# allenai/satlas-super-resolution

Hardware: AMD Instinct MI355X
Metric: G+D train-step images/sec (higher is better)
Workload: dtype fp32h

## Files before the change

### satlas_super_resolution_amd/csrc/conv_x3r.hip

```cpp
#include "conv_x3r_core.h"
#include "conv_dispatch.h"

#ifdef SSR_PROBE
#define RPROBE(cond, k) do { if (cond) g_probe[(blockIdx.y * gridDim.x + blockIdx.x) * 16 + (k)] = __builtin_amdgcn_s_memtime(); } while (0)
#else
#define RPROBE(cond, k)
#endif

namespace {

template <int NTW, int NU, int EP, int TH = 8, int AM = 0>
__global__ __launch_bounds__((XrT<NTW, NU, TH>::NTHR)) void conv_x3r_kernel(const ssr_conv_desc d) {
    constexpr bool EX = AM == 1, H = AM == 2;
    using T = XrT<NTW, NU, TH>;
    constexpr int NT = NTW, NTT = T::NTT, NMF = T::NMF, BN = T::BN, WR = T::WR, MT = T::MT;
    constexpr int G_NPIX = T::NPIX, G_SUB = T::SUB, G_PV = T::PV, G_NPV = T::NPV;
    extern __shared__ __attribute__((aligned(16))) char smem[];
    int* ctl = reinterpret_cast<int*>(smem + T::CTL);
    const int ctl_addr = (int)(size_t)(__attribute__((address_space(3))) char*)(smem + T::CTL);
    const int tid = threadIdx.x, lane = tid & 63, wave = __builtin_amdgcn_readfirstlane(tid >> 6);
    const int tiles_x = (d.Gw + 15) / 16, tiles_y = (d.Gh + TH - 1) / TH;
    int b = blockIdx.x;
    const int tx_i = b % tiles_x; b /= tiles_x;
    const int ty_i = b % tiles_y;
    const int n = b / tiles_y;
    const int gy0 = ty_i * TH, gx0 = tx_i * 16;
    const int co0 = blockIdx.y * BN;
    const int Cin = d.Cin, Cin2 = d.Cin2;
    const int nchunks = (Cin + Cin2 + 15) / 16;
    const int cout_pad = d.CoutPad;
    const int tapstride = cout_pad * 64, wchunk = 9 * tapstride;
    RPROBE(tid == 0, 0);
    if (tid < 4 + NMF) ctl[tid] = 0;
    __syncthreads();

    f32x16 acc[MT][NT];
#pragma unroll
    for (int t = 0; t < MT; ++t)
#pragma unroll
        for (int u = 0; u < NT; ++u)
#pragma unroll
            for (int r = 0; r < 16; ++r) acc[t][u][r] = 0.f;

    if (wave >= NMF) {
        const int pw = wave - NMF;
        const int pt = tid - 64 * NMF;
#ifdef XR_PRIO
        __builtin_amdgcn_s_setprio(3);
#endif
        const int part = pt & 3, p4 = pt >> 2;
        int ppix[G_NPV];
#pragma unroll
        for (int q = 0; q < G_NPV; ++q) {
            const int pix = p4 + 64 * q;
            const int py = pix / XR_PW, px = pix - py * XR_PW;
            const int ly = gy0 + py - d.pad_y, lx = gx0 + px - d.pad_x;
            const bool okp = pix < G_NPIX && ly >= 0 && ly < d.Hi && lx >= 0 && lx < d.Wi;
            ppix[q] = okp ? (n * d.Hi + ly) * d.Wi + lx : -1;
        }
        const int plo0 = p4 * XR_ROWB + part * 8;
        const long xbytes = (long)d.N * d.Hi * d.Wi * 4;
        const void* xp = d.x.p;
        const void* x2p = d.x2.p ? d.x2.p : d.x.p;
        const int x_cs = d.x.cs, x_coff = d.x.coff, x2_cs = d.x2.p ? d.x2.cs : d.x.cs, x2_coff = d.x2.p ? d.x2.coff : d.x.coff;
        u32x4 rq[XR_PQ][G_NPV];
        auto load_chunk = [&](int c, auto jc) {
            constexpr int j = decltype(jc)::value;
            const bool live = c < nchunks;
            const int c0 = c * 16;
            const bool in_x = c0 < Cin;
            const int cb = in_x ? c0 : c0 - Cin, clim = live ? (in_x ? Cin : Cin2) : 0;
            const int cs = in_x ? x_cs : x2_cs, coff = in_x ? x_coff : x2_coff;
            const __amdgpu_buffer_rsrc_t rs = xr_rsrc(in_x ? xp : x2p, xbytes * cs);
            const int k = cb + part * 4;
#pragma unroll
            for (int q = 0; q < G_NPV; ++q) {
                const int off = (ppix[q] * cs + coff + k) * 4;
                const bool okl = (k < clim) & (ppix[q] >= 0);
#ifdef XR_X_NOXLOAD
                rq[j][q] = u32x4{(unsigned)off, (unsigned)okl, 0u, 0u};
#else
                rq[j][q] = __builtin_amdgcn_raw_buffer_load_b128(rs, okl ? off : XR_OOB, 0, 0);
#endif
            }
        };
        static_for<0, XR_PQ>([&](auto jc) { __builtin_amdgcn_sched_barrier(0); load_chunk(decltype(jc)::value, jc); __builtin_amdgcn_sched_barrier(0); });
        RPROBE(pt == 0, 8);
        int cfree = XR_NS;
        for (int c0 = 0; c0 < nchunks; c0 += XR_PQ) {
            static_for<0, XR_PQ>([&](auto jc) {
                constexpr int j = decltype(jc)::value;
                const int c = c0 + j;
                if (c < nchunks) {
                    if (c >= cfree) {
                        int spin = 0;
                        for (; spin < XR_SPIN_MAX; ++spin) {
                            cfree = xr_minN<NMF>(ctl_addr + 16) + XR_NS;
                            if (c < cfree) break;
                            __builtin_amdgcn_s_sleep(2);
                        }
                        if (spin == XR_SPIN_MAX) __builtin_trap();
                    }
                    char* base = smem + (c % XR_NS) * G_SUB;
#pragma unroll
                    for (int q = 0; q < G_NPV; ++q) {
#ifdef XR_X_NOSTORE
                        asm volatile("" :: "v"(rq[j][q]));
                        continue;
#endif
                        if constexpr (EX) {
                            if (q < G_NPV - 1 || pt < G_PV - (G_NPV - 1) * 256)
                                *reinterpret_cast<u32x4*>(base + p4 * XR_ROWB + part * 16 + q * 64 * XR_ROWB) = rq[j][q];
                        } else {
                            uint2 hi, lo;
                            split_f32x4<H>(rq[j][q], hi, lo);
                            if (q < G_NPV - 1 || pt < G_PV - (G_NPV - 1) * 256) {
                                *reinterpret_cast<uint2*>(base + plo0 + q * 64 * XR_ROWB) = hi;
                                *reinterpret_cast<uint2*>(base + plo0 + q * 64 * XR_ROWB + 32) = lo;
                            }
                        }
                    }
                    asm volatile("" ::: "memory");
                    if (lane == 0) *(xr_lds_int)(uintptr_t)(ctl_addr + 4 * pw) = c + 1;
                    asm volatile("" ::: "memory");
#if defined(XR_PRIO) && XR_PRIO == 1
                    if (c == 0) __builtin_amdgcn_s_setprio(0);
#endif
                }
                __builtin_amdgcn_sched_barrier(0);
                load_chunk(c + XR_PQ, jc);
                __builtin_amdgcn_sched_barrier(0);
            });
        }
        RPROBE(pt == 0, 9);
    } else {
        const int w = wave & 3, ug = wave >> 2;
        const int i = lane & 31, gq = lane >> 5;
        const int a_lane = ((i >> 4) * XR_PW + epi_col<XR_ROT>(i)) * XR_ROWB + gq * 16;
        const __amdgpu_buffer_rsrc_t rsw = xr_rsrc(d.w, (long)nchunks * wchunk);
        const int w_lane = (co0 + 32 * NTW * ug + i) * 64 + gq * 16;
        const int nitems = 3 * nchunks;
        const int nj = nitems > w ? (nitems - w + 3) / 4 : 0;
        const int glast = w + 4 * (nj - 1);
        if (nj == 0) {
            if (lane == 0) *(xr_lds_int)(uintptr_t)(ctl_addr + 16 + 4 * wave) = 0x3fffffff;
        } else {
            bf16x8 wf[WR][NT][2];
            constexpr int TPS = T::TPS, SPT = T::SPT, NSUB = 3 * SPT, NSETS = T::NSETS, PD = NSETS - 1;
            bf16x8 af[NSETS][TPS][2];
            auto load_w = [&](int g_, auto kxc, auto sc) {
                constexpr int kx = decltype(kxc)::value, s = decltype(sc)::value;
                const int gg = g_ < glast ? g_ : glast;
                const int c = gg / 3, ky = gg - 3 * c;
                const int off = c * wchunk + (ky * 3 + kx) * tapstride + w_lane;
#pragma unroll
                for (int u = 0; u < NT; ++u) {
                    wf[s][u][0] = __builtin_bit_cast(bf16x8, __builtin_amdgcn_raw_buffer_load_b128(rsw, off + u * 2048, 0, 0));
                    wf[s][u][1] = __builtin_bit_cast(bf16x8, __builtin_amdgcn_raw_buffer_load_b128(rsw, off + u * 2048 + 32, 0, 0));
                }
            };
            auto issue_a = [&](int base, auto qc, auto sc, auto hc) {
                constexpr int q = decltype(qc)::value, kx = q / SPT, part = q % SPT, s = decltype(sc)::value, H = decltype(hc)::value;
#pragma unroll
                for (int t2 = 0; t2 < TPS; ++t2)
                    af[s][t2][H] = *reinterpret_cast<const bf16x8*>(smem + base + kx * XR_ROWB + (part * TPS + t2) * XR_TILEB + 32 * H);
            };
            int avail = 0;
            auto ensure = [&](int c) {
                if (avail > c) return;
                int spin = 0;
                for (; spin < XR_SPIN_MAX; ++spin) {
                    avail = xr_min4(ctl_addr);
                    if (avail > c) break;
                    __builtin_amdgcn_s_sleep(1);
                }
                if (spin == XR_SPIN_MAX) __builtin_trap();
            };
            auto base_of = [&](int g_) { const int c = g_ / 3, ky = g_ - 3 * c; return (c % XR_NS) * G_SUB + ky * XR_PW * XR_ROWB + a_lane; };
            using I0 = std::integral_constant<int, 0>;
            using I1 = std::integral_constant<int, 1>;
#ifndef XR_WPRE
#define XR_WPRE 99
#endif
            constexpr int WPRE = XR_WPRE < WR ? XR_WPRE : WR;
            static_for<0, WPRE>([&](auto sc) {
                constexpr int s = decltype(sc)::value;
                __builtin_amdgcn_sched_barrier(0);
                load_w(w + 4 * (s / 3), std::integral_constant<int, s % 3>{}, sc);
                __builtin_amdgcn_sched_barrier(0);
            });
            RPROBE(tid == 0, 1);
            int g = w, c_cur = g / 3;
            int base_cur = base_of(g);
            ensure(c_cur);
            static_for<WPRE, WR>([&](auto sc) {
                constexpr int s = decltype(sc)::value;
                __builtin_amdgcn_sched_barrier(0);
                load_w(w + 4 * (s / 3), std::integral_constant<int, s % 3>{}, sc);
                __builtin_amdgcn_sched_barrier(0);
            });
            RPROBE(tid == 0, 2);
            static_for<0, PD>([&](auto qc) {
                issue_a(base_cur, qc, std::integral_constant<int, decltype(qc)::value % NSETS>{}, I1{});
                issue_a(base_cur, qc, std::integral_constant<int, decltype(qc)::value % NSETS>{}, I0{});
            });
            int gn = g + 4 < glast ? g + 4 : glast;
            int c_next = gn / 3, base_next = base_of(gn);
            int gnn = gn, c_nn = c_next, base_nn = base_next;
            auto body = [&](int j, auto jpc) {
                constexpr int JP = decltype(jpc)::value;
                static_for<0, NSUB>([&](auto qc) {
                    constexpr int q = decltype(qc)::value, kx = q / SPT, part = q % SPT, qn = q + PD;
                    constexpr int ws = (JP * 3 + kx) % WR, as = (JP * NSUB + q) % NSETS, asn = (JP * NSUB + qn) % NSETS;
                    auto group = [&](auto pc) {
                        constexpr int P = decltype(pc)::value;
                        if constexpr (EX) {
                            constexpr int H = P == 0 ? 1 : 0, S0 = P == 2 ? 2 : 0, S1 = P == 1 ? 2 : 4;
#pragma unroll
                            for (int sidx = S0; sidx < S1; ++sidx)
#pragma unroll
                                for (int t2 = 0; t2 < TPS; ++t2)
#pragma unroll
                                    for (int u = 0; u < NT; ++u) {
                                        const f32x4 av = __builtin_bit_cast(f32x4, af[as][t2][H]), bv = __builtin_bit_cast(f32x4, wf[ws][u][H]);
                                        acc[part * TPS + t2][u] = __builtin_amdgcn_mfma_f32_32x32x2f32(av[sidx], bv[sidx], acc[part * TPS + t2][u], 0, 0, 0);
                                    }
                        } else {
#pragma unroll
                            for (int t2 = 0; t2 < TPS; ++t2)
#pragma unroll
                                for (int u = 0; u < NT; ++u)
                                    acc[part * TPS + t2][u] = split_mfma<H>(af[as][t2][P == 0 ? 1 : 0], wf[ws][u][P == 1 ? 1 : 0], acc[part * TPS + t2][u]);
                        }
                    };
                    auto reads = [&](auto hc) {
#ifndef XR_X_NOA
                        if constexpr (qn < NSUB) issue_a(base_cur, std::integral_constant<int, qn>{}, std::integral_constant<int, asn>{}, hc);
                        else issue_a(base_next, std::integral_constant<int, qn - NSUB>{}, std::integral_constant<int, asn>{}, hc);
#endif
                    };
                    __builtin_amdgcn_sched_barrier(0);
                    if constexpr (qn == NSUB) {
                        if (c_next > c_cur) {
                            asm volatile("" ::: "memory");
                            if (lane == 0) *(xr_lds_int)(uintptr_t)(ctl_addr + 16 + 4 * wave) = c_next;
                            asm volatile("" ::: "memory");
                        }
                        ensure(c_next);
                        __builtin_amdgcn_sched_barrier(0);
                    }
                    group(std::integral_constant<int, 0>{});
                    __builtin_amdgcn_sched_barrier(0);
                    reads(I1{});
                    if constexpr (part == 0) {
#ifndef XR_X_NOW
                        constexpr int wsp = (JP * 3 + kx + WR - 1) % WR, ioff = (kx + WR - 1) / 3, tap = (kx + WR - 1) % 3;
                        load_w(g + 4 * ioff, std::integral_constant<int, tap>{}, std::integral_constant<int, wsp>{});
#endif
                    }
                    __builtin_amdgcn_sched_barrier(0);
                    group(std::integral_constant<int, 1>{});
                    __builtin_amdgcn_sched_barrier(0);
                    reads(I0{});
                    if constexpr (q == 0) {
                        gnn = g + 8 < glast ? g + 8 : glast;
                        c_nn = gnn / 3;
                        base_nn = base_of(gnn);
                    }
                    __builtin_amdgcn_sched_barrier(0);
                    group(std::integral_constant<int, 2>{});
                    __builtin_amdgcn_sched_barrier(0);
                });
                g += 4;
                c_cur = c_next; base_cur = base_next;
                gn = gnn; c_next = c_nn; base_next = base_nn;
#ifdef SSR_PROBE
                if (j < 5) RPROBE(tid == 0, 3 + j);
#endif
            };
            if constexpr (WR == 6 || (NSUB % NSETS) != 0) {
                for (int j = 0; j < nj; j += 2) {
                    body(j, std::integral_constant<int, 0>{});
                    if (j + 1 < nj) body(j + 1, std::integral_constant<int, 1>{});
                }
            } else {
                for (int j = 0; j < nj; ++j) body(j, std::integral_constant<int, 0>{});
            }
            asm volatile("" ::: "memory");
            if (lane == 0) *(xr_lds_int)(uintptr_t)(ctl_addr + 16 + 4 * wave) = 0x3fffffff;
        }
    }
    __syncthreads();
    RPROBE(tid == 0, 10);

    const bool is_mfma = wave < NMF;
    const int me = is_mfma ? (wave & 3) : wave - NMF;
    const int ut = is_mfma ? NTW * (wave >> 2) : 1;
#ifndef XR_X_NORED
    if (is_mfma) {
#pragma unroll
        for (int t = 0; t < MT; ++t)
#pragma unroll
            for (int u = 0; u < NT; ++u)
                if (!(t == me && u == 0)) {
                    char* sp = smem + ((me * MT + t) * NTT + ut + u) * XR_SLOT + lane * 16;
#pragma unroll
                    for (int q = 0; q < 4; ++q) {
                        f32x4 v = {acc[t][u][4 * q], acc[t][u][4 * q + 1], acc[t][u][4 * q + 2], acc[t][u][4 * q + 3]};
                        *reinterpret_cast<f32x4*>(sp + q * 1024) = v;
                    }
                }
    }
#endif
    __syncthreads();
    if ((is_mfma || NTW == 2) && me < MT) {
        f32x16 own;
#pragma unroll
        for (int r = 0; r < 16; ++r) own[r] = 0.f;
        if (is_mfma) {
#pragma unroll
            for (int t = 0; t < MT; ++t)
                if (t == me) own = acc[t][0];
        }
        f32x16 sum;
#pragma unroll
        for (int s = 0; s < 4; ++s) {
            f32x16 part;
            const char* sp = smem + ((s * MT + me) * NTT + ut) * XR_SLOT + lane * 16;
#ifdef XR_X_NORED
            part = own;
            asm volatile("" : "+v"(part));
#else
#pragma unroll
            for (int q = 0; q < 4; ++q) {
                const f32x4 v = *reinterpret_cast<const f32x4*>(sp + q * 1024);
                part[4 * q] = v[0]; part[4 * q + 1] = v[1]; part[4 * q + 2] = v[2]; part[4 * q + 3] = v[3];
            }
#endif
            const bool mine = is_mfma && s == me;
#pragma unroll
            for (int r = 0; r < 16; ++r) {
                const float p = mine ? own[r] : part[r];
                sum[r] = s == 0 ? p : sum[r] + p;
            }
        }
        if constexpr (H) {
#pragma unroll
            for (int r = 0; r < 16; ++r) sum[r] *= SSR_F32H_UNSCALE;
        }
        char* slab = smem + (((is_mfma ? me : 0) * MT + me) * NTT + ut) * XR_SLOT;
        const int cb = co0 + 32 * ut;
#ifdef XR_X_NOEPI
        float keep = 0.f;
#pragma unroll
        for (int r = 0; r < 16; ++r) keep += sum[r];
        if (keep == 123.456f) reinterpret_cast<float*>(d.y.p)[tid] = keep;
#else
        if constexpr (EP == XR_EP_GENERIC) conv_epilogue<float, XR_ROT>(d, sum, cb, n, gy0 + 2 * me, gx0, lane, slab);
        else xr_epilogue<EP>(d, sum, cb, n, gy0 + 2 * me, gx0, lane, slab);
#endif
    }
    RPROBE(tid == 0, 11);
}

template <int NTW, int NU, int EP, int TH = 8, int AM = 0>
int launch_x3r(const ssr_conv_desc& d, hipStream_t st) {
    using T = XrT<NTW, NU, TH>;
    auto kern = conv_x3r_kernel<NTW, NU, EP, TH, AM>;
    static bool attr_done[SSR_MAX_DEVICES] = {};
    const int dev = ssr_device_ordinal();
    if (!attr_done[dev]) {
        hipError_t e = hipFuncSetAttribute(reinterpret_cast<const void*>(kern), hipFuncAttributeMaxDynamicSharedMemorySize, T::LDS);
        if (e != hipSuccess) return (int)e;
        attr_done[dev] = true;
    }
    const int tiles = ((d.Gw + 15) / 16) * ((d.Gh + TH - 1) / TH) * d.N;
    hipLaunchKernelGGL(kern, dim3(tiles, d.CoutPad / T::BN, 1), dim3(T::NTHR), T::LDS, st, d);
    SSR_LAUNCH_CHECK();
    return SSR_OK;
}

int xr_pick_epilogue(const ssr_conv_desc& d) {
    static const bool generic_only = ssr_env_off("SSR_X3R_EPI");
    if (generic_only) return XR_EP_GENERIC;
    const long lim = 0x7fffff00L, npx = (long)d.N * d.Ho * d.Wo * 4;
    auto vok = [&](const ssr_view& v) { return (v.cs % 4) == 0 && (v.coff % 4) == 0 && ((uintptr_t)v.p % 16) == 0 && npx * v.cs <= lim; };
    if (d.fix_list || d.y0.p || d.y1.p || d.accumulate || d.m_relu || (d.Cout % 4) != 0 || !vok(d.y)) return XR_EP_GENERIC;
    if (d.oys != 1 || d.oxs != 1 || d.oyo != 0 || d.oxo != 0 || d.Ho < d.Gh || d.Wo < d.Gw) return XR_EP_GENERIC;
    const bool r1 = d.r1.p != nullptr, r2 = d.r2.p != nullptr, m = d.m.p != nullptr;
    if (d.act == SSR_ACT_LRELU && d.alpha == 1.f && !r1 && !r2 && !m) return XR_EP_LRELU;
    if (d.act == SSR_ACT_NONE && !m && (!r1 || (d.r1_nc >= d.Cout && vok(d.r1))) && (!r2 || (d.r2_nc >= d.Cout && vok(d.r2)))) return XR_EP_LIN;
    if (d.act == SSR_ACT_NONE && d.alpha == 1.f && m && !r1 && !r2 && d.m_c0 == 0 && d.m_c1 >= d.Cout && vok(d.m)) return XR_EP_MASK;
    return XR_EP_GENERIC;
}

template <int NTW, int NU, int TH = 8, int AM = 0>
int launch_x3r_ep(const ssr_conv_desc& d, hipStream_t st) {
    switch (xr_pick_epilogue(d)) {
        case XR_EP_LRELU: return launch_x3r<NTW, NU, XR_EP_LRELU, TH, AM>(d, st);
        case XR_EP_LIN: return launch_x3r<NTW, NU, XR_EP_LIN, TH, AM>(d, st);
        case XR_EP_MASK: return launch_x3r<NTW, NU, XR_EP_MASK, TH, AM>(d, st);
        default: return launch_x3r<NTW, NU, XR_EP_GENERIC, TH, AM>(d, st);
    }
}

int xr_tile_height(const ssr_conv_desc& d, int form) {
    static const int forced = ssr_env_int("SSR_X3_REGTILE_TH", 0);
    if (form != 0) return 8;
    if (forced == 4 || forced == 8) return forced;
    const long tiles8 = (long)((d.Gw + 15) / 16) * ((d.Gh + 7) / 8) * d.N * (d.CoutPad / 32);
    return (tiles8 <= 160 && d.Gh > 4) ? 4 : 8;
}

int xr_wide_form(const ssr_conv_desc& d) {
    static const int f = ssr_env_off("SSR_X3_REGTILE_NT2") ? 0 : ssr_env_int("SSR_X3_REGTILE_NT2", 1) == 8 ? 2 : 1;
    if ((d.CoutPad % 64) != 0) return 0;
    static const bool split_off = ssr_env_off("SSR_X3_REGTILE_SPLIT");
    const long tiles = (long)((d.Gw + 15) / 16) * ((d.Gh + 7) / 8) * d.N;
    if (!split_off && tiles * (d.CoutPad / 64) <= 160) return 0;
    return (f == 2 && xr_pick_epilogue(d) == XR_EP_GENERIC) ? 1 : f;
}

bool x3r_shape_ok(const ssr_conv_desc& d) {
    static const bool ex_off = ssr_env_off("SSR_F32_REGTILE");
    if (!(d.dtype == SSR_F32X3 || d.dtype == SSR_F32H || (d.dtype == SSR_F32 && !ex_off)) || d.fix_list) return false;
    if (d.dtype == SSR_F32 && (d.act == SSR_ACT_RELU || d.m_relu)) return false;
    if (!(d.KH == 3 && d.KW == 3 && d.stride == 1 && d.pad_y == 1 && d.pad_x == 1 && d.up == 1 && !d.s2d)) return false;
    if (d.Gh != d.Hi || d.Gw != d.Wi || (d.CoutPad % 32) != 0) return false;
    if (d.x2.p && (d.Cin % 16) != 0) return false;
    const long lim = 0x7fffff00L, npx = (long)d.N * d.Hi * d.Wi * 4;
    if (npx * d.x.cs > lim || (d.x2.p && npx * d.x2.cs > lim)) return false;
    if ((long)((d.Cin + d.Cin2 + 15) / 16) * 9 * d.CoutPad * 64 > lim) return false;
    return true;
}

bool x3r_qualifies(const ssr_conv_desc& d) {
    static const bool off = ssr_env_off("SSR_X3_REGTILE");
    if (off || !x3r_shape_ok(d)) return false;
    return d.Gh <= 64 && d.Gw <= 64 && d.Cin + d.Cin2 >= 16;
}

template <int AM>
int launch_x3r_am(const ssr_conv_x3r_instance& i, const ssr_conv_desc& d, hipStream_t st) {
    if constexpr (AM == 0)
        if (i.nu == 2) return launch_x3r_ep<1, 2>(d, st);
    if (i.ntw == 2) return launch_x3r_ep<2, 1, 8, AM>(d, st);
    return i.th == 4 ? launch_x3r_ep<1, 1, 4, AM>(d, st) : launch_x3r_ep<1, 1, 8, AM>(d, st);
}

int x3r_launch(const ssr_conv_desc& d, hipStream_t st) {
    const ssr_conv_x3r_instance i = ssr_conv_x3r_pick(d);
    return i.am == 1 ? launch_x3r_am<1>(i, d, st) : i.am == 2 ? launch_x3r_am<2>(i, d, st) : launch_x3r_am<0>(i, d, st);
}

int x3r_code(const ssr_conv_desc& d) { return ((d.CoutPad % 64) == 0 ? 2 : 1) * 10 + 5; }
void x3r_symbol(const ssr_conv_desc& d, int, char* buf, int buflen) {
    const ssr_conv_x3r_instance i = ssr_conv_x3r_pick(d);
    snprintf(buf, buflen, "conv_x3r_kernel<%d, %d, %d, %d, %d>", i.ntw, i.nu, i.ep, i.th, i.am);
}

}

ssr_conv_x3r_instance ssr_conv_x3r_pick(const ssr_conv_desc& d) {
    const int am = d.dtype == SSR_F32 ? 1 : d.dtype == SSR_F32H ? 2 : 0;
    int f = xr_wide_form(d);
    if (am != 0 && f == 2) f = 1;
    return {f == 1 ? 2 : 1, f == 2 ? 2 : 1, xr_pick_epilogue(d), xr_tile_height(d, f), am};
}

ssr_conv_family ssr_conv_x3r = {"x3r", 7, x3r_shape_ok, x3r_qualifies, x3r_launch, x3r_code, x3r_symbol};
```

### satlas_super_resolution_amd/csrc/conv_x3r_core.h

```cpp
#pragma once
#include "conv_epilogue.h"
#include <cstdlib>

namespace {

constexpr int XR_NMFMA = 4, XR_NPROD = 4, XR_NTHR = 64 * (XR_NMFMA + XR_NPROD);
constexpr int XR_ROWB = 80, XR_PH = 10, XR_PW = 18, XR_NPIX = XR_PH * XR_PW;
constexpr int XR_SUB = XR_NPIX * XR_ROWB;
constexpr int XR_NS = 8;
constexpr int XR_RING = XR_NS * XR_SUB;
constexpr int XR_PV = XR_NPIX * 4;
constexpr int XR_NPV = (XR_PV + 255) / 256;
#ifndef XR_PQ_DEPTH
#define XR_PQ_DEPTH 4
#endif
constexpr int XR_PQ = XR_PQ_DEPTH;
constexpr int XR_ROT = 14;
constexpr int XR_OOB = 0x7ffffff0;
constexpr int XR_SPIN_MAX = 1 << 22;
constexpr int XR_TILEB = 2 * XR_PW * XR_ROWB;
constexpr int XR_SLOT = 32 * 32 * 4;

template <int NTW, int NU = 1, int TH = 8> struct XrT {
    static_assert(TH == 8 || TH == 4, "tile height");
    static constexpr int MT = TH / 2;
    static constexpr int PH = TH + 2, NPIX = PH * XR_PW;
    static constexpr int SUB = NPIX * XR_ROWB;
    static constexpr int RING = XR_NS * SUB;
    static constexpr int PV = NPIX * 4, NPV = (PV + 255) / 256;
    static constexpr int NTT = NTW * NU;
    static constexpr int BN = 32 * NTT;
    static constexpr int NMF = 4 * NU;
    static constexpr int NTHR = 64 * (NMF + 4);
    static constexpr int WR = (NTW == 1 && NU == 1) ? 6 : 3;
#ifndef XR_TPS1
#define XR_TPS1 4
#endif
    static constexpr int TPS = (NTW == 1 ? XR_TPS1 : 2) < MT ? (NTW == 1 ? XR_TPS1 : 2) : MT;
    static constexpr int SPT = MT / TPS;
    static constexpr int NSETS = SPT == 1 ? 2 : 3;
    static constexpr int SLOTS = 4 * MT * NTT;
    static constexpr int RED = SLOTS * XR_SLOT;
    static constexpr int CTL = RED > RING ? RED : RING;
    static constexpr int LDS = CTL + 256;
    static_assert(LDS <= 160 * 1024, "LDS budget");
};

__device__ __forceinline__ __amdgpu_buffer_rsrc_t xr_rsrc(const void* p, long bytes) {
    return __builtin_amdgcn_make_buffer_rsrc(const_cast<void*>(p), 0, (int)(bytes > 0x7fffff00L ? 0x7fffff00L : (bytes < 0 ? 0 : bytes)), 0x00020000);
}
__device__ __forceinline__ void xr_split4(const u32x4& v, uint2& hi, uint2& lo) {
    const f32x4 f = __builtin_bit_cast(f32x4, v);
    bf16x4 h, l;
#pragma unroll
    for (int k = 0; k < 4; ++k) {
        h[k] = (__bf16)f[k];
        l[k] = (__bf16)(f[k] - (float)h[k]);
    }
    hi = __builtin_bit_cast(uint2, h);
    lo = __builtin_bit_cast(uint2, l);
}
typedef __attribute__((address_space(3))) int* xr_lds_int;

__device__ __forceinline__ int xr_min4(int a) {
    u32x4 v;
    asm volatile("ds_read_b128 %0, %1\n\ts_waitcnt lgkmcnt(0)" : "=&v"(v) : "v"(a) : "memory");
    return __builtin_amdgcn_readfirstlane((int)min(min(v[0], v[1]), min(v[2], v[3])));
}

template <int N> __device__ __forceinline__ int xr_minN(int a) {
    if constexpr (N == 4) return xr_min4(a);
    else {
        u32x4 v, w;
        asm volatile("ds_read_b128 %0, %2\n\tds_read_b128 %1, %2 offset:16\n\ts_waitcnt lgkmcnt(0)" : "=&v"(v), "=&v"(w) : "v"(a) : "memory");
        const unsigned m = min(min(min(v[0], v[1]), min(v[2], v[3])), min(min(w[0], w[1]), min(w[2], w[3])));
        return __builtin_amdgcn_readfirstlane((int)m);
    }
}

enum { XR_EP_LRELU = 0, XR_EP_LIN = 1, XR_EP_MASK = 2, XR_EP_GENERIC = 3 };

template <int EP, int AUX = 0>
__device__ __forceinline__ void xr_epilogue(const ssr_conv_desc& d, const f32x16& acc, int co_base, int n, int gy_row0, int gx0, int lane,
                                             char* slab) {
    const int i = lane & 31, g = lane >> 5;
    const int part = lane & 7, c = co_base + part * 4;
    const bool cok = c < d.Cout;
    const long npix = (long)d.N * d.Ho * d.Wo * 4;
    const __amdgpu_buffer_rsrc_t rs_y = xr_rsrc(d.y.p, npix * d.y.cs);
    int pp[4];
    bool ok[4];
#pragma unroll
    for (int h = 0; h < 4; ++h) {
        const int pix = (lane >> 3) + 8 * h;
        const int gy = gy_row0 + (pix >> 4), gx = gx0 + epi_col<XR_ROT>(pix);
        ok[h] = cok && gy < d.Gh && gx < d.Gw;
        pp[h] = (n * d.Ho + gy) * d.Wo + gx;
    }
    f32x4 bv = {0.f, 0.f, 0.f, 0.f};
    if (d.bias) {
        const __amdgpu_buffer_rsrc_t rs_b = xr_rsrc(d.bias, (long)d.Cout * 4);
#pragma unroll
        for (int k = 0; k < 4; ++k) bv[k] = __builtin_bit_cast(float, __builtin_amdgcn_raw_buffer_load_b32(rs_b, (c + k) * 4, 0, 0));
    }
    u32x4 q1[4], q2[4];
    if constexpr (EP == XR_EP_LIN) {
        const __amdgpu_buffer_rsrc_t rs_r1 = xr_rsrc(d.r1.p, d.r1.p ? npix * d.r1.cs : 0), rs_r2 = xr_rsrc(d.r2.p, d.r2.p ? npix * d.r2.cs : 0);
        const bool h1 = d.r1.p != nullptr, h2 = d.r2.p != nullptr;
#pragma unroll
        for (int h = 0; h < 4; ++h) {
            q1[h] = __builtin_amdgcn_raw_buffer_load_b128(rs_r1, ok[h] && h1 ? (pp[h] * d.r1.cs + d.r1.coff + c) * 4 : XR_OOB, 0, 0);
            q2[h] = __builtin_amdgcn_raw_buffer_load_b128(rs_r2, ok[h] && h2 ? (pp[h] * d.r2.cs + d.r2.coff + c) * 4 : XR_OOB, 0, 0);
        }
    }
    if constexpr (EP == XR_EP_MASK) {
        const __amdgpu_buffer_rsrc_t rs_m = xr_rsrc(d.m.p, npix * d.m.cs);
#pragma unroll
        for (int h = 0; h < 4; ++h) q1[h] = __builtin_amdgcn_raw_buffer_load_b128(rs_m, ok[h] ? (pp[h] * d.m.cs + d.m.coff + c) * 4 : XR_OOB, 0, 0);
    }
    float* sl = reinterpret_cast<float*>(slab);
#pragma unroll
    for (int r = 0; r < 16; ++r) sl[mfma32_row(r, g) * 32 + i] = acc[r];
    const float alpha = d.alpha, beta1 = d.beta1, beta2 = d.beta2;
#pragma unroll
    for (int h = 0; h < 4; ++h) {
        const int pix = (lane >> 3) + 8 * h;
        f32x4 v = *reinterpret_cast<const f32x4*>(sl + pix * 32 + part * 4);
        if constexpr (EP == XR_EP_LRELU) {
#pragma unroll
            for (int k = 0; k < 4; ++k) v[k] = lrelu_max(v[k] + bv[k]);
        } else if constexpr (EP == XR_EP_LIN) {
            const f32x4 a = __builtin_bit_cast(f32x4, q1[h]), b = __builtin_bit_cast(f32x4, q2[h]);
#pragma unroll
            for (int k = 0; k < 4; ++k) v[k] = alpha * (v[k] + bv[k]) + (beta1 * a[k] + beta2 * b[k]);
        } else {
            const f32x4 m = __builtin_bit_cast(f32x4, q1[h]);
#pragma unroll
            for (int k = 0; k < 4; ++k) v[k] = (v[k] + bv[k]) * lrelu_grad_from_out(m[k]);
        }
        __builtin_amdgcn_raw_buffer_store_b128(__builtin_bit_cast(u32x4, v), rs_y, ok[h] ? (pp[h] * d.y.cs + d.y.coff + c) * 4 : XR_OOB, 0, AUX);
    }
}

}
```

Baseline: 1186.

## Prefetch epilogue operands early and distribute split-K reduction across all threads

```diff
diff --git a/satlas_super_resolution_amd/csrc/conv_x3r.hip b/satlas_super_resolution_amd/csrc/conv_x3r.hip
--- a/satlas_super_resolution_amd/csrc/conv_x3r.hip
+++ b/satlas_super_resolution_amd/csrc/conv_x3r.hip
@@ -42,6 +42,25 @@
 #pragma unroll
             for (int r = 0; r < 16; ++r) acc[t][u][r] = 0.f;
 
+    constexpr bool ITEMS = EP != XR_EP_GENERIC;
+    constexpr int OPS_EARLY = (NTW == 1 && NU == 1) ? ((TH == 8 || EP == XR_EP_LRELU) ? 2 : 1) : 0;
+    constexpr int NITEMS = MT * NTT * 256, NIT = ITEMS ? (NITEMS + T::NTHR - 1) / T::NTHR : 1;
+    XrItemOps ops[NIT];
+    auto fetch_ops = [&](auto pc) {
+        if constexpr (ITEMS) {
+            __builtin_amdgcn_sched_barrier(0);
+#pragma unroll
+            for (int k = 0; k < NIT; ++k) {
+                const int it = tid + T::NTHR * k, tl = it >> 8, pix = (it >> 3) & 31;
+                xr_item_fetch<EP, decltype(pc)::value>(d, co0 + 32 * (tl % NTT) + 4 * (it & 7), n, gy0 + 2 * (tl / NTT) + (pix >> 4),
+                                                       gx0 + epi_col<XR_ROT>(pix), it < NITEMS, ops[k]);
+            }
+            __builtin_amdgcn_sched_barrier(0);
+        }
+    };
+    using P0 = std::integral_constant<int, 0>;
+    using P1 = std::integral_constant<int, 1>;
+
     if (wave >= NMF) {
         const int pw = wave - NMF;
         const int pt = tid - 64 * NMF;
@@ -133,6 +152,8 @@
             });
         }
         RPROBE(pt == 0, 9);
+        fetch_ops(P0{});
+        fetch_ops(P1{});
     } else {
         const int w = wave & 3, ug = wave >> 2;
         const int i = lane & 31, gq = lane >> 5;
@@ -144,6 +165,8 @@
         const int glast = w + 4 * (nj - 1);
         if (nj == 0) {
             if (lane == 0) *(xr_lds_int)(uintptr_t)(ctl_addr + 16 + 4 * wave) = 0x3fffffff;
+            fetch_ops(P0{});
+            fetch_ops(P1{});
         } else {
             bf16x8 wf[WR][NT][2];
             constexpr int TPS = T::TPS, SPT = T::SPT, NSUB = 3 * SPT, NSETS = T::NSETS, PD = NSETS - 1;
@@ -189,6 +212,8 @@
                 load_w(w + 4 * (s / 3), std::integral_constant<int, s % 3>{}, sc);
                 __builtin_amdgcn_sched_barrier(0);
             });
+            if constexpr (OPS_EARLY >= 1) fetch_ops(P0{});
+            if constexpr (OPS_EARLY >= 2) fetch_ops(P1{});
             RPROBE(tid == 0, 1);
             int g = w, c_cur = g / 3;
             int base_cur = base_of(g);
@@ -288,77 +313,119 @@
             }
             asm volatile("" ::: "memory");
             if (lane == 0) *(xr_lds_int)(uintptr_t)(ctl_addr + 16 + 4 * wave) = 0x3fffffff;
+            if constexpr (OPS_EARLY < 1) fetch_ops(P0{});
+            if constexpr (OPS_EARLY < 2) fetch_ops(P1{});
         }
     }
     __syncthreads();
     RPROBE(tid == 0, 10);
 
-    const bool is_mfma = wave < NMF;
-    const int me = is_mfma ? (wave & 3) : wave - NMF;
-    const int ut = is_mfma ? NTW * (wave >> 2) : 1;
+    if constexpr (ITEMS) {
 #ifndef XR_X_NORED
-    if (is_mfma) {
-#pragma unroll
-        for (int t = 0; t < MT; ++t)
-#pragma unroll
-            for (int u = 0; u < NT; ++u)
-                if (!(t == me && u == 0)) {
-                    char* sp = smem + ((me * MT + t) * NTT + ut + u) * XR_SLOT + lane * 16;
-#pragma unroll
-                    for (int q = 0; q < 4; ++q) {
-                        f32x4 v = {acc[t][u][4 * q], acc[t][u][4 * q + 1], acc[t][u][4 * q + 2], acc[t][u][4 * q + 3]};
-                        *reinterpret_cast<f32x4*>(sp + q * 1024) = v;
+        if (wave < NMF) {
+            char* sp = smem + ((wave & 3) * MT * NTT + NTW * (wave >> 2)) * XR_SLOT + (lane >> 5) * 512 + (lane & 31) * 4;
+#pragma unroll
+            for (int t = 0; t < MT; ++t)
+#pragma unroll
+                for (int u = 0; u < NT; ++u)
+#pragma unroll
+                    for (int r = 0; r < 16; ++r)
+                        *reinterpret_cast<float*>(sp + (t * NTT + u) * XR_SLOT + mfma32_row(r, 0) * 128) = acc[t][u][r];
+        }
+#endif
+        __syncthreads();
+#pragma unroll
+        for (int k = 0; k < NIT; ++k) {
+            const int it = tid + T::NTHR * k;
+            if ((NITEMS % T::NTHR) == 0 || it < NITEMS) {
+                const char* rp = smem + (it >> 8) * XR_SLOT + (it & 255) * 16;
+                f32x4 v = *reinterpret_cast<const f32x4*>(rp);
+#pragma unroll
+                for (int s = 1; s < 4; ++s) {
+                    const f32x4 p = *reinterpret_cast<const f32x4*>(rp + s * MT * NTT * XR_SLOT);
+#pragma unroll
+                    for (int e = 0; e < 4; ++e) v[e] += p[e];
+                }
+                if constexpr (H) {
+#pragma unroll
+                    for (int e = 0; e < 4; ++e) v[e] *= SSR_F32H_UNSCALE;
+                    asm volatile("" : "+v"(v));
+                }
+#ifdef XR_X_NOEPI
+                const float keep = (v[0] + v[1]) + (v[2] + v[3]);
+                if (keep == 123.456f) reinterpret_cast<float*>(d.y.p)[tid] = keep;
+#else
+                xr_item_finish<EP>(d, v, ops[k]);
+#endif
+            }
+        }
+    } else {
+        const bool is_mfma = wave < NMF;
+        const int me = is_mfma ? (wave & 3) : wave - NMF;
+        const int ut = is_mfma ? NTW * (wave >> 2) : 1;
+#ifndef XR_X_NORED
+        if (is_mfma) {
+#pragma unroll
+            for (int t = 0; t < MT; ++t)
+#pragma unroll
+                for (int u = 0; u < NT; ++u)
+                    if (!(t == me && u == 0)) {
+                        char* sp = smem + ((me * MT + t) * NTT + ut + u) * XR_SLOT + lane * 16;
+#pragma unroll
+                        for (int q = 0; q < 4; ++q) {
+                            f32x4 v = {acc[t][u][4 * q], acc[t][u][4 * q + 1], acc[t][u][4 * q + 2], acc[t][u][4 * q + 3]};
+                            *reinterpret_cast<f32x4*>(sp + q * 1024) = v;
+                        }
                     }
-                }
-    }
-#endif
-    __syncthreads();
-    if ((is_mfma || NTW == 2) && me < MT) {
-        f32x16 own;
-#pragma unroll
-        for (int r = 0; r < 16; ++r) own[r] = 0.f;
-        if (is_mfma) {
-#pragma unroll
-            for (int t = 0; t < MT; ++t)
-                if (t == me) own = acc[t][0];
-        }
-        f32x16 sum;
-#pragma unroll
-        for (int s = 0; s < 4; ++s) {
-            f32x16 part;
-            const char* sp = smem + ((s * MT + me) * NTT + ut) * XR_SLOT + lane * 16;
+        }
+#endif
+        __syncthreads();
+        if ((is_mfma || NTW == 2) && me < MT) {
+            f32x16 own;
+#pragma unroll
+            for (int r = 0; r < 16; ++r) own[r] = 0.f;
+            if (is_mfma) {
+#pragma unroll
+                for (int t = 0; t < MT; ++t)
+                    if (t == me) own = acc[t][0];
+            }
+            f32x16 sum;
+#pragma unroll
+            for (int s = 0; s < 4; ++s) {
+                f32x16 part;
+                const char* sp = smem + ((s * MT + me) * NTT + ut) * XR_SLOT + lane * 16;
 #ifdef XR_X_NORED
-            part = own;
-            asm volatile("" : "+v"(part));
+                part = own;
+                asm volatile("" : "+v"(part));
 #else
 #pragma unroll
-            for (int q = 0; q < 4; ++q) {
-                const f32x4 v = *reinterpret_cast<const f32x4*>(sp + q * 1024);
-                part[4 * q] = v[0]; part[4 * q + 1] = v[1]; part[4 * q + 2] = v[2]; part[4 * q + 3] = v[3];
-            }
-#endif
-            const bool mine = is_mfma && s == me;
-#pragma unroll
-            for (int r = 0; r < 16; ++r) {
-                const float p = mine ? own[r] : part[r];
-                sum[r] = s == 0 ? p : sum[r] + p;
-            }
-        }
-        if constexpr (H) {
-#pragma unroll
-            for (int r = 0; r < 16; ++r) sum[r] *= SSR_F32H_UNSCALE;
-        }
-        char* slab = smem + (((is_mfma ? me : 0) * MT + me) * NTT + ut) * XR_SLOT;
-        const int cb = co0 + 32 * ut;
+                for (int q = 0; q < 4; ++q) {
+                    const f32x4 v = *reinterpret_cast<const f32x4*>(sp + q * 1024);
+                    part[4 * q] = v[0]; part[4 * q + 1] = v[1]; part[4 * q + 2] = v[2]; part[4 * q + 3] = v[3];
+                }
+#endif
+                const bool mine = is_mfma && s == me;
+#pragma unroll
+                for (int r = 0; r < 16; ++r) {
+                    const float p = mine ? own[r] : part[r];
+                    sum[r] = s == 0 ? p : sum[r] + p;
+                }
+            }
+            if constexpr (H) {
+#pragma unroll
+                for (int r = 0; r < 16; ++r) sum[r] *= SSR_F32H_UNSCALE;
+            }
+            char* slab = smem + (((is_mfma ? me : 0) * MT + me) * NTT + ut) * XR_SLOT;
+            const int cb = co0 + 32 * ut;
 #ifdef XR_X_NOEPI
-        float keep = 0.f;
-#pragma unroll
-        for (int r = 0; r < 16; ++r) keep += sum[r];
-        if (keep == 123.456f) reinterpret_cast<float*>(d.y.p)[tid] = keep;
+            float keep = 0.f;
+#pragma unroll
+            for (int r = 0; r < 16; ++r) keep += sum[r];
+            if (keep == 123.456f) reinterpret_cast<float*>(d.y.p)[tid] = keep;
 #else
-        if constexpr (EP == XR_EP_GENERIC) conv_epilogue<float, XR_ROT>(d, sum, cb, n, gy0 + 2 * me, gx0, lane, slab);
-        else xr_epilogue<EP>(d, sum, cb, n, gy0 + 2 * me, gx0, lane, slab);
-#endif
+            conv_epilogue<float, XR_ROT>(d, sum, cb, n, gy0 + 2 * me, gx0, lane, slab);
+#endif
+        }
     }
     RPROBE(tid == 0, 11);
 }
diff --git a/satlas_super_resolution_amd/csrc/conv_x3r_core.h b/satlas_super_resolution_amd/csrc/conv_x3r_core.h
--- a/satlas_super_resolution_amd/csrc/conv_x3r_core.h
+++ b/satlas_super_resolution_amd/csrc/conv_x3r_core.h
@@ -142,4 +142,54 @@
     }
 }
 
+struct XrItemOps {
+    f32x4 bv;
+    u32x4 q1, q2;
+    int yoff;
+};
+
+template <int EP, int PART>
+__device__ __forceinline__ void xr_item_fetch(const ssr_conv_desc& d, int c, int n, int gy, int gx, bool live, XrItemOps& o) {
+    const long npix = (long)d.N * d.Ho * d.Wo * 4;
+    const bool ok = live && c < d.Cout && gy < d.Gh && gx < d.Gw;
+    const int pp = (n * d.Ho + gy) * d.Wo + gx;
+    if constexpr (PART == 0) {
+        if constexpr (EP == XR_EP_LIN) {
+            const __amdgpu_buffer_rsrc_t rs_r1 = xr_rsrc(d.r1.p, d.r1.p ? npix * d.r1.cs : 0);
+            o.q1 = __builtin_amdgcn_raw_buffer_load_b128(rs_r1, ok && d.r1.p ? (pp * d.r1.cs + d.r1.coff + c) * 4 : XR_OOB, 0, 0);
+        }
+        if constexpr (EP == XR_EP_MASK) {
+            const __amdgpu_buffer_rsrc_t rs_m = xr_rsrc(d.m.p, npix * d.m.cs);
+            o.q1 = __builtin_amdgcn_raw_buffer_load_b128(rs_m, ok ? (pp * d.m.cs + d.m.coff + c) * 4 : XR_OOB, 0, 0);
+        }
+    } else {
+        o.yoff = ok ? (pp * d.y.cs + d.y.coff + c) * 4 : XR_OOB;
+        const __amdgpu_buffer_rsrc_t rs_b = xr_rsrc(d.bias, d.bias ? (long)d.Cout * 4 : 0);
+        o.bv = __builtin_bit_cast(f32x4, __builtin_amdgcn_raw_buffer_load_b128(rs_b, c * 4, 0, 0));
+        if constexpr (EP == XR_EP_LIN) {
+            const __amdgpu_buffer_rsrc_t rs_r2 = xr_rsrc(d.r2.p, d.r2.p ? npix * d.r2.cs : 0);
+            o.q2 = __builtin_amdgcn_raw_buffer_load_b128(rs_r2, ok && d.r2.p ? (pp * d.r2.cs + d.r2.coff + c) * 4 : XR_OOB, 0, 0);
+        }
+    }
 }
+
+template <int EP, int AUX = 0>
+__device__ __forceinline__ void xr_item_finish(const ssr_conv_desc& d, f32x4 v, const XrItemOps& o) {
+    const __amdgpu_buffer_rsrc_t rs_y = xr_rsrc(d.y.p, (long)d.N * d.Ho * d.Wo * 4 * d.y.cs);
+    const float alpha = d.alpha, beta1 = d.beta1, beta2 = d.beta2;
+    if constexpr (EP == XR_EP_LRELU) {
+#pragma unroll
+        for (int k = 0; k < 4; ++k) v[k] = lrelu_max(v[k] + o.bv[k]);
+    } else if constexpr (EP == XR_EP_LIN) {
+        const f32x4 a = __builtin_bit_cast(f32x4, o.q1), b = __builtin_bit_cast(f32x4, o.q2);
+#pragma unroll
+        for (int k = 0; k < 4; ++k) v[k] = __builtin_fmaf(alpha, v[k] + o.bv[k], __builtin_fmaf(beta1, a[k], beta2 * b[k]));
+    } else {
+        const f32x4 m = __builtin_bit_cast(f32x4, o.q1);
+#pragma unroll
+        for (int k = 0; k < 4; ++k) v[k] = (v[k] + o.bv[k]) * lrelu_grad_from_out(m[k]);
+    }
+    __builtin_amdgcn_raw_buffer_store_b128(__builtin_bit_cast(u32x4, v), rs_y, o.yoff, 0, AUX);
+}
+
+}
```

Measured after the change: 1219 (median of 6 runs). 1.03x the previous value.
